# intellerce/controlanimate

Measured on AMD Instinct MI355X. Metric: frames_per_sec, higher is better.
Workload: dtype fp16

## Files before the change

controlanimate_amd/_capi.py:

```python
from __future__ import annotations

import ctypes as C
import os

_HERE = os.path.dirname(os.path.abspath(__file__))
LIB_PATH = os.environ.get("CA_HIP_LIB") or os.path.join(_HERE, "csrc", "libcontrolanimate_hip.so")

CA_BF16, CA_F16 = 0, 1
CA_F32 = 2
CA_ACT_NONE, CA_ACT_SILU = 0, 1
ABI_VERSION = 16


class CAHipUnavailable(RuntimeError):
    pass


class CAHipError(RuntimeError):
    pass


class GemmArgs(C.Structure):
    _fields_ = [
        ("a", C.c_void_p), ("a2", C.c_void_p), ("w", C.c_void_p), ("c", C.c_void_p),
# ... 162 lines not shown
                                         C.c_void_p, C.c_void_p, C.c_int32, C.c_int32, C.c_int32, C.c_int32,
                                         C.POINTER(C.c_float), C.c_float, C.c_void_p]),
    "ca_lincomb": (C.c_int, [C.c_void_p, C.POINTER(C.c_void_p), C.POINTER(C.c_float), C.c_int32, C.c_int64, C.c_void_p]),
    "ca_conv3x3_narrow": (C.c_int, [C.POINTER(ConvNarrowArgs), C.c_void_p]),
    "ca_conv3x3_narrow_plan_name": (C.c_int, [C.POINTER(ConvNarrowArgs), C.c_char_p, C.c_int32]),
    "ca_rgb8_to_nhwc": (C.c_int, [C.c_void_p, C.c_void_p, C.c_int32, C.c_int32, C.c_int32, C.c_int32, C.c_void_p]),
    "ca_resize_lanczos4_u8": (C.c_int, [C.c_void_p, C.c_void_p, C.c_int32, C.c_int32, C.c_int32, C.c_int32, C.c_int32,
                                         C.c_void_p, C.c_void_p, C.c_void_p, C.c_void_p, C.c_void_p]),
    "ca_color_match_workspace_bytes": (C.c_int64, [C.c_int32, C.c_int64]),
    "ca_hist_u8x3": (C.c_int, [C.c_void_p, C.c_void_p, C.c_int32, C.c_int64, C.c_void_p]),
    "ca_color_moments_f64": (C.c_int, [C.c_void_p, C.c_void_p, C.c_void_p, C.c_void_p, C.c_int32, C.c_int64, C.c_void_p, C.c_int64, C.c_void_p]),
    "ca_color_transform_f64": (C.c_int, [C.c_void_p, C.c_void_p, C.c_void_p, C.c_void_p, C.c_void_p, C.c_void_p, C.c_int32, C.c_int64, C.c_void_p]),
    "ca_sort_f64_segments": (C.c_int, [C.c_void_p, C.c_void_p, C.c_int32, C.c_int64, C.c_void_p, C.c_int64, C.c_void_p]),
    "ca_color_rank_map_f64": (C.c_int, [C.c_void_p, C.c_void_p, C.c_void_p, C.c_void_p, C.c_void_p, C.c_void_p, C.c_int32, C.c_int64,
                                         C.c_void_p, C.c_int64, C.c_void_p]),
    "ca_color_finish_u8": (C.c_int, [C.c_void_p, C.c_void_p, C.c_int32, C.c_int64, C.c_int32, C.c_void_p, C.c_int64, C.c_void_p]),
    "ca_canny_workspace_bytes": (C.c_int64, [C.c_int32, C.c_int32, C.c_int32]),
    "ca_canny_tile_w": (C.c_int32, []),
    "ca_canny_tile_h": (C.c_int32, []),
    "ca_canny_classify": (C.c_int, [C.c_void_p, C.c_int32, C.c_int32, C.c_int32, C.c_int32, C.c_int32, C.c_int32, C.c_void_p, C.c_int64, C.c_void_p]),
    "ca_canny_link": (C.c_int, [C.c_int32, C.c_int32, C.c_int32, C.c_void_p, C.c_int64, C.c_void_p]),
    "ca_canny_link_stage": (C.c_int, [C.c_int32, C.c_int32, C.c_int32, C.c_void_p, C.c_int64, C.c_int32, C.c_void_p]),
    "ca_canny_emit": (C.c_int, [C.c_int32, C.c_int32, C.c_int32, C.c_void_p, C.c_int64, C.c_void_p, C.c_void_p, C.c_int32, C.c_int32, C.c_void_p]),
}

_lib = None


def lib() -> C.CDLL:
    global _lib
    if _lib is not None:
        return _lib
    import torch
    if not os.path.exists(LIB_PATH):
        raise CAHipUnavailable(
            f"{LIB_PATH} is missing: the HIP extension is not built. Run "
            "`python -m controlanimate_amd._build` (needs hipcc); there is no CPU fallback.")
    try:
        handle = C.CDLL(LIB_PATH)
    except OSError as e:
        raise CAHipUnavailable(f"cannot load {LIB_PATH}: {e}") from e
    for name, (res, args) in SYMBOLS.items():
        fn = getattr(handle, name)
        fn.restype = res
        fn.argtypes = args
    if handle.ca_abi_version() != ABI_VERSION:
# ... 10 lines not shown
```

controlanimate_amd/context.py:

```python
from __future__ import annotations

from dataclasses import dataclass, field
from typing import Optional

import torch


@dataclass
class ExecCtx:
    b: int
    f: int
    dtype: torch.dtype
    temb: torch.Tensor
    emb_groups: int
    ehs: Optional[torch.Tensor] = None
    frames_per_kv: int = 1
    kv_mod: int = 0
    gn_frames_per_stat: int = 1
    cache: dict = field(default_factory=dict)

    @property
    def images(self) -> int:
        return self.b * self.f

    def rows_per_emb_group(self, h: int, w: int) -> int:
        return self.images // self.emb_groups * h * w


class Dispatch:
    gemm_ar = True
    ff_fused = True
    tattn_fused = True
    xattn_fused = True
    attn_out_fused = True
    xattn_ip_fused = True
    conv_winograd = True
    gn_winograd = True
    ln_row_sums = True
    repeat_kernel = True
    ln_fold = True
    cfg_shared = True
    cn_cfg_dedup = True
    controlnet_streams = 2


dispatch = Dispatch()
```

controlanimate_amd/csrc/ca_gemm.hip:

```cpp

#include "ca_gemm_core.h"

namespace {
using namespace ca_gemm_detail;
#include "ca_conv_wino.h"

template <int DT, int BM, int BN, int WAVES_M, int WAVES_N, int MODE>
__global__ __launch_bounds__(256) void k_gemm(GemmKParams p) {
  constexpr int TM = BM / WAVES_M / 16;
  constexpr int TN = BN / WAVES_N / 16;
  constexpr int AI = BM / 32;
  constexpr int BI = BN / 32;
  static_assert(2 * (BM + BN) * BK >= BM * (BN + 8), "epilogue staging must fit");
  __shared__ __attribute__((aligned(16))) u16 smem[2 * (BM + BN) * BK];

  const int tid = threadIdx.x;
  const int lane = tid & 63;
  const int wid = tid >> 6;
  const int wm = wid / WAVES_N, wn = wid % WAVES_N;
  const int g = lane >> 4, l15 = lane & 15;

  const int tiles_n = (p.n + BN - 1) / BN;
  const unsigned bid = xcd_remap(blockIdx.x, gridDim.x);
  int tile_m, tile_n;
// ... 875 lines not shown
  return CA_OK;
}

extern "C" int ca_conv3x3(const ca_conv_args* a, void* stream) {
  GemmKParams p{};
  int rc = conv_prepare(a, p);
  if (rc) return rc;
  hipStream_t st = (hipStream_t)stream;
  if (wino_taken(a)) {
    rc = launch_conv_wino(a, p, st);
    if (rc) return rc;
    CA_CHECK_LAUNCH("ca_conv3x3(winograd)");
    return CA_OK;
  }
  CA_REQUIRE(!a->x_is_wino_v, "ca_conv3x3: x_is_wino_v, but the Winograd route does not take these arguments (images=%d %dx%d cin=%d+%d cout=%d dtype=%d w_wino=%p "
             "workspace=%p of %lld bytes, needs %lld)", a->images, a->hin, a->win, a->cin1, a->cin2, a->cout, a->dtype, a->w_wino, a->workspace,
             (long long)a->workspace_bytes, (long long)wino_workspace_bytes(a));
  rc = a->dtype == CA_BF16 ? launch_gemm<CA_BF16, 1>(p, st) : launch_gemm<CA_F16, 1>(p, st);
  if (rc) return rc;
  CA_CHECK_LAUNCH("ca_conv3x3");
  return CA_OK;
}

extern "C" int ca_gemm_plan_name(const ca_gemm_args* a, char* buf, int32_t len) {
  CA_REQUIRE(buf && len > 0, "ca_gemm_plan_name: buffer");
  GemmKParams p{};
  int rc = gemm_prepare(a, p);
  if (rc) return rc;
  plan_label(plan_gemm(p, 0), buf, len);
  return CA_OK;
}

extern "C" int ca_conv3x3_plan_name(const ca_conv_args* a, char* buf, int32_t len) {
  CA_REQUIRE(buf && len > 0, "ca_conv3x3_plan_name: buffer");
  GemmKParams p{};
  int rc = conv_prepare(a, p);
  if (rc) return rc;
  if (wino_taken(a)) {
    snprintf(buf, (size_t)len, "wino_pq256x320");
    return CA_OK;
  }
  plan_label(plan_gemm(p, 1), buf, len);
  return CA_OK;
}
```

controlanimate_amd/csrc/ca_gemm_core.h:

```cpp
#pragma once
#include "ca_common.h"
#include <stdlib.h>

namespace ca_gemm_detail {


struct GemmKParams {
  const u16* a;
  const u16* a2;
  const u16* w;
  void* c;
  const float* bias;
  const float* rowbias;
  const float* ln_stats;
  const float* ln_colsum;
  const u16* res;
  int64_t lda, lda2, ldc, ld_res, ld_rowbias;
  unsigned a_bytes, a2_bytes, w_bytes;
  int m, n;
  int c1, c2;
  int taps;
  int kc_tiles;
  int hin, win, hout, wout, stride, ups, pad_lo;
  int rows_per_group;
  float alpha, post;
  int act, geglu, out_f32;
  int splits;
  float* partial;
  int dbg;
  int tap_inner;
  float* row_sums;
  int ln_parts;
  int ln_inline;
  float ln_eps;
  const u16* wf;
  int w_group_rows;
  unsigned w_group_stride;
};

constexpr int BK = 64;

constexpr int GROUP_M = 8;
__device__ __forceinline__ void tile_coords(unsigned bid, int tiles_m, int tiles_n, int& tile_m, int& tile_n) {
  const unsigned gsz = GROUP_M * tiles_n;
  const unsigned group = bid / gsz, in = bid - group * gsz;
  const int first_m = group * GROUP_M;
  const int gm = tiles_m - first_m < GROUP_M ? tiles_m - first_m : GROUP_M;
  tile_m = first_m + in % gm;
  tile_n = in / gm;
}

__device__ __forceinline__ void k_tile_split(const GemmKParams& p, int t, int kct, int& tap, int& cc) {
  if (p.taps == 1) {
    tap = 0;
    cc = t;
  } else if (p.tap_inner) {
    cc = t / p.taps;
    tap = t - cc * p.taps;
  } else {
    tap = t / kct;
// ... 281 lines not shown
        b += v.y;
      }
      *reinterpret_cast<float2*>(p.row_sums + ((int64_t)(m0 + tid) * (p.n / BN) + n0 / BN) * 2) = make_float2(a, b);
    }
  }
}


constexpr unsigned DMA_OOB = 0xFFFFFFF0u;

enum PlanKind {
  PK_WRES = 0,
  PK_PP2,
  PK_PP2_SPLITK,
  PK_DMA,
  PK_DMA_SPLITK,
  PK_REG,
  PK_PS,
  PK_PQ,
  PK_AR,
};

constexpr int64_t FIT31 = 0x7FFFFF00ll;
inline int64_t c_extent_bytes(const GemmKParams& p) { return (((int64_t)p.m - 1) * p.ldc + (p.geglu ? p.n / 2 : p.n)) * 2; }
inline int64_t res_extent_bytes(const GemmKParams& p) { return p.res ? (((int64_t)p.m - 1) * p.ld_res + p.n) * 2 : 0; }
inline bool act_out_fit31(const GemmKParams& p) {
  return c_extent_bytes(p) < FIT31 && res_extent_bytes(p) < FIT31 && p.a_bytes < FIT31 && (!p.c2 || p.a2_bytes < FIT31);
}

}

int ca_launch_gemm_pp(const ca_gemm_detail::GemmKParams& p, int dtype, int mode, ca_gemm_detail::PlanKind kind, unsigned tiles, hipStream_t st);
int ca_launch_gemm_ar(const ca_gemm_detail::GemmKParams& p, int dtype, hipStream_t st);
```

controlanimate_amd/csrc/ca_gemm_pp.hip:

```cpp
#include "ca_gemm_core.h"
#include <type_traits>

namespace {
using namespace ca_gemm_detail;
#include "ca_gemm_pp2.h"
#include "ca_gemm_wres.h"
#include "ca_gemm_ps.h"
#include "ca_gemm_pq.h"

int cu_count() {
  static int n = 0;
  if (!n) {
    int dev = 0;
    hipDeviceProp_t prop;
    if (hipGetDevice(&dev) == hipSuccess && hipGetDeviceProperties(&prop, dev) == hipSuccess) n = prop.multiProcessorCount;
    if (n <= 0) n = 256;
  }
  return n;
}

template <class Launch>
int launch_stamped(const GemmKParams& p, hipStream_t st, const char* label, unsigned sep, unsigned eol, Launch launch) {
  static unsigned long long* dbuf = nullptr;
  if (!dbuf && hipMalloc(&dbuf, 4096 * 8) != hipSuccess) return CA_ERR_LAUNCH;
// ... 43 lines not shown
#ifdef CA_STAMPS
      if (p.dbg == 9) return launch_stamped(p, st, "ps", 8, 10, launch);
#endif
      launch(p);
      return CA_OK;
    }
    case PK_WRES: {
      if (MODE != 0) return CA_ERR_LAUNCH;
      const int panels = p.n / 160;
      const int chunks = (p.m + 255) / 256;
      int per = (cu_count() / 8) / panels;
      if (per * 8 > chunks) per = chunks / 8;
      if (per < 1) per = 1;
      const unsigned rb_bytes = p.rowbias ? (unsigned)(((int64_t)((p.m - 1) / p.rows_per_group) * p.ld_rowbias + p.n) * 4) : 16u;
      hipLaunchKernelGGL((k_gemm_wres<DT>), dim3(8 * per * panels), dim3(512), 0, st, p, panels, 8 * per, chunks, rb_bytes, c_bytes, res_bytes);
      return CA_OK;
    }
    case PK_PP2:
      hipLaunchKernelGGL((k_gemm_pp2<DT, MODE>), dim3(tiles), dim3(512), 0, st, p);
      return CA_OK;
    default: return CA_ERR_LAUNCH;
  }
}
}

int ca_launch_gemm_pp(const ca_gemm_detail::GemmKParams& p0, int dtype, int mode, ca_gemm_detail::PlanKind kind, unsigned tiles, hipStream_t st) {
  static const int dbg = CA_KNOB("CA_PP_DBG", 0);
  ca_gemm_detail::GemmKParams p = p0;
  p.dbg = dbg;
  if (dtype == CA_BF16) return mode ? launch_pp<CA_BF16, 1>(p, kind, tiles, st) : launch_pp<CA_BF16, 0>(p, kind, tiles, st);
  return mode ? launch_pp<CA_F16, 1>(p, kind, tiles, st) : launch_pp<CA_F16, 0>(p, kind, tiles, st);
}
```

controlanimate_amd/csrc/ca_gemm_pq.h:

```cpp

#ifdef CA_PQ_ABLATE
#define CA_PQ_ABL(bit) (((CA_PQ_ABLATE) & (bit)) != 0)
#else
#define CA_PQ_ABL(bit) false
#endif

template <int DT, int MODE, int EPI = 0>
__global__ __launch_bounds__(512, 2) void k_gemm_pq(GemmKParams p, int tiles_total, unsigned c_bytes, unsigned res_bytes) {
  constexpr int BM = 256, BN = 320, KT = 64;
  constexpr int TM = 8, TN = 5;
  constexpr int A_ROWS = 256, B0_ROWS = 128, B1_ROWS = 192;
  constexpr int OFF_A = 0, OFF_B0 = A_ROWS * KT, OFF_B1 = (A_ROWS + B0_ROWS) * KT;
  constexpr int BUF = (A_ROWS + B0_ROWS + B1_ROWS) * KT;
  constexpr int PAR_BASE = 2 * BUF * 2;
  constexpr int P_BI = 0, P_RB0 = 1280, P_RB1 = 2560, P_CS = 3840, PSET = EPI == 1 ? 5120 : 4096;
  constexpr int FLAG_BASE = PAR_BASE + 2 * PSET;
  constexpr int SMEM_BYTES = FLAG_BASE + 8 * 2 * 256;
  static_assert(SMEM_BYTES <= 160 * 1024, "LDS");
  __shared__ __attribute__((aligned(16))) unsigned char smem_b[SMEM_BYTES];
  u16* const smem = reinterpret_cast<u16*>(smem_b);

  const int tid = threadIdx.x;
  const int lane = tid & 63;
  const int wid = __builtin_amdgcn_readfirstlane(tid >> 6);
  const int wr = wid >> 2, wc = wid & 3;
  const int g = lane >> 4, l15 = lane & 15;

  const int tiles_n = p.n / BN;
  const int tiles_m = (p.m + BM - 1) / BM;
  const int G = gridDim.x;
  const int bslot = (G % 8 == 0) ? (int)(blockIdx.x % 8) * (G / 8) + (int)(blockIdx.x / 8) : (int)blockIdx.x;
  const int my_tiles = bslot < tiles_total ? (tiles_total - bslot + G - 1) / G : 0;
  if (my_tiles == 0) return;

  for (int i = tid; i < 8 * 2 * 64; i += 512) reinterpret_cast<unsigned*>(smem_b + FLAG_BASE)[i] = 0xFFFFFFFFu;
  __syncthreads();

  const __amdgpu_buffer_rsrc_t rs_a = __builtin_amdgcn_make_buffer_rsrc((void*)p.a, 0, p.a_bytes, 0x00020000);
  const __amdgpu_buffer_rsrc_t rs_a2 = __builtin_amdgcn_make_buffer_rsrc((void*)(p.a2 ? p.a2 : p.a), 0, p.a2 ? p.a2_bytes : p.a_bytes, 0x00020000);
  const __amdgpu_buffer_rsrc_t rs_w = __builtin_amdgcn_make_buffer_rsrc((void*)p.w, 0, p.w_bytes, 0x00020000);
  const __amdgpu_buffer_rsrc_t rs_c = __builtin_amdgcn_make_buffer_rsrc(p.c, 0, c_bytes, 0x00020000);
  const __amdgpu_buffer_rsrc_t rs_bi = __builtin_amdgcn_make_buffer_rsrc((void*)(p.bias ? (const void*)p.bias : (const void*)p.w), 0, p.bias ? (unsigned)p.n * 4u : 0u, 0x00020000);
  const bool geglu = EPI == 1 && p.geglu != 0;
  const unsigned long long res_addr = (unsigned long long)(p.res ? (const void*)p.res : (const void*)p.c);
  const u32x4 rs_res = {(unsigned)__builtin_amdgcn_readfirstlane((int)(unsigned)res_addr), (unsigned)__builtin_amdgcn_readfirstlane((int)(unsigned)((res_addr >> 32) & 0xffffu)),
                        (unsigned)__builtin_amdgcn_readfirstlane((int)(p.res ? res_bytes : 0u)), 0x00020000u};
  const unsigned rb_groups = p.rowbias ? (unsigned)((p.m + p.rows_per_group - 1) / p.rows_per_group) : 0u;
  const __amdgpu_buffer_rsrc_t rs_rb = __builtin_amdgcn_make_buffer_rsrc((void*)(p.rowbias ? (const void*)p.rowbias : (const void*)p.w), 0,
                                                                         p.rowbias ? (unsigned)(((int64_t)(rb_groups - 1) * p.ld_rowbias + p.n) * 4) : 0u, 0x00020000);
  const __amdgpu_buffer_rsrc_t rs_seq = __builtin_amdgcn_make_buffer_rsrc((void*)ca_seq_table.v, 0, 4096u, 0x00020000);

#ifdef CA_STAMPS
// ... 20 lines not shown
  unsigned b0_v[2] = {0, 0}, b1_v[3] = {0, 0, 0};
  unsigned a_v[4] = {0, 0, 0, 0};
  int d_seq = 0, d_t = 0, d_tap = 0, d_c0 = 0, d_n = 0;
  bool d_live = true;
  unsigned char* const my_flags = smem_b + FLAG_BASE + wid * 2 * 256;

  auto tile_of = [&](int seq, int& tm, int& tn) __attribute__((always_inline)) -> bool {
    const int id = seq * G + bslot;
    if (id >= tiles_total) return false;
    tile_coords((unsigned)id, tiles_m, tiles_n, tm, tn);
    return true;
  };

  auto dma_set_tile = [&](int seq, int m0, int n0) __attribute__((always_inline)) {
    if (CA_PQ_ABL(16)) m0 = 0, n0 = 0;
    int lane_o = lane;
    asm volatile("" : "+v"(lane_o));
    const int r8 = lane_o >> 3, cp = lane_o & 7;
    const int a_chunk0 = cp ^ swz(r8), b1_chunk0 = cp ^ swz(wid * 24 + r8);
#pragma unroll
    for (int i = 0; i < 4; ++i) {
      const int m = m0 + wid * 32 + i * 8 + r8;
      const bool ok = m < p.m;
      if (MODE == 1) {
        const int mm = ok ? m : p.m - 1;
        const int hw = p.hout * p.wout;
        const int img = mm / hw;
        const int rem = mm - img * hw;
        const int ho = rem / p.wout, wo = rem - ho * p.wout;
        const int hi0 = ho * p.stride - p.pad_lo, wi0 = wo * p.stride - p.pad_lo;
        const int p0 = (img * p.hin + hi0) * p.win + wi0;
        a_v[i] = ((unsigned)p0 & 0xFFFFFFu) | (hi0 >= 0 ? 1u << 24 : 0u) | (hi0 + 2 < p.hin ? 1u << 25 : 0u) | (wi0 >= 0 ? 1u << 26 : 0u) | (wi0 + 2 < p.win ? 1u << 27 : 0u) |
                 (ok ? 1u << 28 : 0u);
      } else {
        a_v[i] = ok ? (unsigned)m * (unsigned)p.lda * 2u + (unsigned)((a_chunk0 ^ (4 * (i & 1))) * 16) : OOB_V;
      }
    }
    unsigned wgrp = 0u;
    if (MODE == 0 && EPI == 0 && p.w_group_rows > 0) wgrp = (unsigned)(m0 / p.w_group_rows) * p.w_group_stride;
#pragma unroll
    for (int i = 0; i < 2; ++i) {
      const int r = wid * 16 + i * 8 + r8;
      b0_v[i] = wgrp + (unsigned)(n0 + (r >> 5) * 80 + ca_ps_col((r >> 4) & 1, r & 15, geglu)) * wld * 2u + (unsigned)((a_chunk0 ^ (4 * i)) * 16);
    }
#pragma unroll
    for (int i = 0; i < 3; ++i) {
      const int r1 = wid * 24 + i * 8 + r8;
      b1_v[i] = wgrp + (unsigned)(n0 + (r1 / 48) * 80 + ca_ps_col(2 + (r1 % 48) / 16, r1 & 15, geglu)) * wld * 2u + (unsigned)((b1_chunk0 ^ (4 * (i & 1))) * 16);
    }
    d_tap = 0;
    d_c0 = 0;
    unsigned char* pset = smem_b + PAR_BASE + (seq & 1) * PSET;
    if (EPI == 1 && wid == 4) {
      const __amdgpu_buffer_rsrc_t rs_cs = __builtin_amdgcn_make_buffer_rsrc((void*)(p.ln_colsum ? (const void*)p.ln_colsum : (const void*)p.w), 0, p.ln_colsum ? (unsigned)p.n * 4u : 0u, 0x00020000);
      __builtin_amdgcn_raw_ptr_buffer_load_lds(rs_cs, (__attribute__((address_space(3))) void*)(pset + P_CS), 16, (unsigned)n0 * 4u + lane_o * 16u, 0, 0, 0);
      __builtin_amdgcn_raw_ptr_buffer_load_lds(rs_cs, (__attribute__((address_space(3))) void*)(pset + P_CS + 1024), 4, (unsigned)n0 * 4u + 1024u + lane_o * 4u, 0, 0, 0);
    }
    if (wid >= 1 && wid <= 3) {
      const bool has1 = p.rowbias && m0 / p.rows_per_group + 1 < (int)rb_groups;
      const unsigned base = wid == 1 ? (unsigned)n0 * 4u
                                     : wid == 2 ? (unsigned)n0 * 4u + (unsigned)(p.rowbias ? m0 / p.rows_per_group : 0) * (unsigned)p.ld_rowbias * 4u
                                                : (has1 ? (unsigned)n0 * 4u + (unsigned)(m0 / p.rows_per_group + 1) * (unsigned)p.ld_rowbias * 4u : OOB_V);
// ... 1 lines not shown
      if (wid == 1) {
        __builtin_amdgcn_raw_ptr_buffer_load_lds(rs_bi, (__attribute__((address_space(3))) void*)dst, 16, base + lane_o * 16u, 0, 0, 0);
        __builtin_amdgcn_raw_ptr_buffer_load_lds(rs_bi, (__attribute__((address_space(3))) void*)(dst + 1024), 4, base + 1024u + lane_o * 4u, 0, 0, 0);
      } else {
        __builtin_amdgcn_raw_ptr_buffer_load_lds(rs_rb, (__attribute__((address_space(3))) void*)dst, 16, base + lane_o * 16u, 0, 0, 0);
        __builtin_amdgcn_raw_ptr_buffer_load_lds(rs_rb, (__attribute__((address_space(3))) void*)(dst + 1024), 4, base + 1024u + lane_o * 4u, 0, 0, 0);
      }
    }
  };

  auto issue_tile = [&]() __attribute__((always_inline)) {
    if (!d_live) return;
    if (CA_PQ_ABL(1) && d_n >= 2) {
      ++d_n;
      ++d_t;
      return;
    }
    const int par = d_n & 1;
    u16* buf = smem + par * BUF;
    const unsigned wk = (unsigned)(d_tap * kc + d_c0) * 2u;
    const bool src2 = d_c0 >= p.c1;
    __builtin_amdgcn_raw_ptr_buffer_load_lds(rs_w, (__attribute__((address_space(3))) void*)(buf + OFF_B0 + (wid * 2 + 0) * 8 * KT), 16, b0_v[0], wk, 0, 0);
    __builtin_amdgcn_raw_ptr_buffer_load_lds(rs_w, (__attribute__((address_space(3))) void*)(buf + OFF_B0 + (wid * 2 + 1) * 8 * KT), 16, b0_v[1], wk, 0, 0);
    if (MODE == 1) {
      int lane_o = lane;
      asm volatile("" : "+v"(lane_o));
      const unsigned cs2 = (unsigned)(src2 ? p.c2 : p.c1) * 2u;
      const int kh = d_tap >= 6 ? 2 : (d_tap >= 3 ? 1 : 0), kw = d_tap - kh * 3;
      const unsigned need = (1u << 28) | (kh == 0 ? 1u << 24 : kh == 2 ? 1u << 25 : 0u) | (kw == 0 ? 1u << 26 : kw == 2 ? 1u << 27 : 0u);
      const int delta = kh * p.win + kw;
      const unsigned cadd = (unsigned)(src2 ? d_c0 - p.c1 : d_c0) * 2u + (unsigned)(((lane_o & 7) ^ swz(lane_o >> 3)) * 16);
#pragma unroll
      for (int i = 0; i < 4; ++i) {
        const unsigned av = a_v[i];
        const int pix = (((int)(av << 8)) >> 8) + delta;
        const unsigned off = __umul24((unsigned)pix, cs2) + (cadd ^ ((i & 1) ? 64u : 0u));
        const unsigned voff = (av & need) == need ? off : OOB_V;
        void* d = buf + OFF_A + (wid * 4 + i) * 8 * KT;
        if (src2) __builtin_amdgcn_raw_ptr_buffer_load_lds(rs_a2, (__attribute__((address_space(3))) void*)d, 16, voff, 0, 0, 0);
        else __builtin_amdgcn_raw_ptr_buffer_load_lds(rs_a, (__attribute__((address_space(3))) void*)d, 16, voff, 0, 0, 0);
      }
    } else {
#pragma unroll
      for (int i = 0; i < 4; ++i)
        __builtin_amdgcn_raw_ptr_buffer_load_lds(rs_a, (__attribute__((address_space(3))) void*)(buf + OFF_A + (wid * 4 + i) * 8 * KT), 16, a_v[i], (unsigned)d_c0 * 2u, 0, 0);
    }
#pragma unroll
    for (int i = 0; i < 3; ++i)
      __builtin_amdgcn_raw_ptr_buffer_load_lds(rs_w, (__attribute__((address_space(3))) void*)(buf + OFF_B1 + (wid * 3 + i) * 8 * KT), 16, b1_v[i], wk, 0, 0);
    __builtin_amdgcn_raw_ptr_buffer_load_lds(rs_seq, (__attribute__((address_space(3))) void*)(my_flags + par * 256), 4, 0u, (unsigned)(d_n & 1023) * 4u, 0, 0);
    ++d_n;
    ++d_t;
// ... 83 lines not shown
#pragma unroll
    for (int i = 0; i < TM; ++i)
#pragma unroll
      for (int j = 0; j < TN; ++j) acc[i][j] = Elem<DT>::mfma(fb[j], fa[i], acc[i][j]);
    __builtin_amdgcn_s_setprio(0);
    __builtin_amdgcn_sched_barrier(0);
  };

  auto epilogue = [&](int seq, int m0, int n0) __attribute__((always_inline)) {
    const unsigned char* pset = smem_b + PAR_BASE + (seq & 1) * PSET;
    int lane_o = lane;
    asm volatile("" : "+v"(lane_o));
    const int l15 = lane_o & 15, g = lane_o >> 4;
    int rb_sel = 0;
    if (p.rowbias) rb_sel = (m0 + wr * 128) / p.rows_per_group - m0 / p.rows_per_group;
    const unsigned char* rbp = pset + (rb_sel ? P_RB1 : P_RB0);
    f32x4 bi[TN], rb[TN];
#pragma unroll
    for (int j = 0; j < TN; ++j) {
      const int c0 = wc * 80 + (j < 4 ? 32 * (j >> 1) + 8 * g + 4 * (j & 1) : 64 + 4 * g);
      bi[j] = *reinterpret_cast<const f32x4*>(pset + P_BI + c0 * 4);
      rb[j] = *reinterpret_cast<const f32x4*>(rbp + c0 * 4);
    }
    auto rowoff_of = [&](int i, int64_t ld) __attribute__((always_inline)) -> unsigned {
      const int m = m0 + wr * 128 + i * 16 + l15;
      return m < p.m ? (unsigned)m * (unsigned)ld * 2u + (unsigned)(n0 + wc * 80) * 2u : OOB_V;
    };
    u32x4 r16[2][2];
    u32x2 r8[2];
    r16[0][0] = r16[0][1] = r16[1][0] = r16[1][1] = (u32x4){0u, 0u, 0u, 0u};
    r8[0] = r8[1] = (u32x2){0u, 0u};
    auto res_load = [&](int i, int slot) __attribute__((always_inline)) {
      const unsigned ro = rowoff_of(i, p.ld_res);
      const unsigned o0 = ro + (unsigned)(8 * g) * 2u, o1 = ro + (unsigned)(32 + 8 * g) * 2u, o2 = ro + (unsigned)(64 + 4 * g) * 2u;
      asm volatile("s_nop 4\n\tbuffer_load_dwordx4 %0, %3, %6, 0 offen\n\tbuffer_load_dwordx4 %1, %4, %6, 0 offen\n\tbuffer_load_dwordx2 %2, %5, %6, 0 offen"
                   : "=&v"(r16[slot][0]), "=&v"(r16[slot][1]), "=&v"(r8[slot])
                   : "v"(o0), "v"(o1), "v"(o2), "s"(rs_res)
                   : "memory");
    };
    float rsum[TM], rsq[TM];
#pragma unroll
    for (int i = 0; i < TM; ++i) rsum[i] = rsq[i] = 0.f;
    if (p.res) res_load(0, 0);
#pragma unroll
    for (int i = 0; i < TM; ++i) {
      const int slot = i & 1;
      if (p.res) {
        if (i + 1 < TM) res_load(i + 1, slot ^ 1);
        if (i == 0 || i + 1 == TM) asm volatile("s_waitcnt vmcnt(3)" ::: "memory");
// ... 106 lines not shown
          const unsigned lo = pack2<DT>(v[0], v[1]), hi = pack2<DT>(v[2], v[3]);
          if ((j & 1) == 0) {
            w[0] = lo;
            w[1] = hi;
          } else {
            __builtin_amdgcn_raw_buffer_store_b128((u32x4){w[0], w[1], lo, hi}, rs_c, ro + (unsigned)(32 * (j >> 1) + 8 * g) * 2u, 0, 0);
          }
        } else {
          __builtin_amdgcn_raw_buffer_store_b64((u32x2){pack2<DT>(v[0], v[1]), pack2<DT>(v[2], v[3])}, rs_c, ro + (unsigned)(64 + 4 * g) * 2u, 0, 0);
        }
      }
      if (geglu) {
        __builtin_amdgcn_raw_buffer_store_b128((u32x4){w[0], w[1], w[2], w[3]}, rs_c, ro + (unsigned)(8 * g) * 2u, 0, 0);
        __builtin_amdgcn_raw_buffer_store_b32(w[4], rs_c, ro + (unsigned)(32 + 2 * g) * 2u, 0, 0);
      }
    }
#pragma unroll
    for (int i = 0; i < TM; ++i)
#pragma unroll
      for (int j = 0; j < TN; ++j) acc[i][j] = (f32x4){0.f, 0.f, 0.f, 0.f};
    asm volatile("s_waitcnt lgkmcnt(0)" ::: "memory");
  };

  const bool g1_late = MODE == 1 && wr == 1;
  CA_PQ_SET_TILE(0)
  issue_tile();
  if (g1_late) advance_and_issue();
  {
    const unsigned f0 = flag_begin(0);
    flag_finish(0, 0, f0);
  }
  __builtin_amdgcn_s_barrier();
  if (wr == 1) __builtin_amdgcn_s_barrier();

  int cv = 0;
  for (int seq = 0; seq < my_tiles; ++seq) {
    int tm, tn;
    tile_of(seq, tm, tn);
    const int m0 = tm * BM, n0 = tn * BN;
    for (int t = 0; t < (p.dbg == 2 ? 0 : nt); ++t) {
      const int par = cv & 1;
      const u16* buf = smem + par * BUF;
      stamp(1);
      __builtin_amdgcn_sched_barrier(0);
      read_frags(buf, 0);
      if (!g1_late) advance_and_issue();
      asm volatile("s_waitcnt lgkmcnt(0)" ::: "memory");
// ... 35 lines not shown
```

controlanimate_amd/kernels.py:

```python
from __future__ import annotations

import ctypes as C
from typing import Optional

import torch

from . import _capi
from .context import dispatch
from ._capi import (AttnArgs, ConvArgs, ConvNarrowArgs, FfArgs, TattnArgs, XattnArgs, GemmArgs, GroupNormArgs, LayerNormArgs, CA_ACT_NONE,
                    CA_ACT_SILU, CA_BF16, CA_F16, check, lib)

ACT_NONE, ACT_SILU = CA_ACT_NONE, CA_ACT_SILU
ACT_QUICK_GELU, ACT_GELU = 2, 3


def dt_code(dtype: torch.dtype) -> int:
    if dtype == torch.bfloat16:
        return CA_BF16
    if dtype == torch.float16:
        return CA_F16
    raise TypeError(f"activations must be bf16 or fp16, got {dtype}")


def _stream() -> int:
# ... 251 lines not shown
        ld_res = cout
    if rowbias is not None:
        assert rowbias.dtype == torch.float32 and rowbias.dim() == 2 and rowbias.shape[1] == cout and rows_per_group > 0
    if bias is not None:
        assert bias.dtype == torch.float32 and bias.numel() == cout
    args = ConvArgs(x=_p(x), x2=_p(x2), w=_p(w), y=_p(y), bias=_p(bias), rowbias=_p(rowbias),
                    residual=_p(residual), ld_res=ld_res,
                    ld_rowbias=rowbias.stride(0) if rowbias is not None else 0, images=images, hin=hin,
                    win=win, cin1=cin1, cin2=cin2, cout=cout, stride=stride, upsample=int(upsample),
                    rows_per_group=rows_per_group, alpha=alpha, post_scale=post_scale, act=act,
                    out_f32=int(out_f32), dtype=dt_code(x.dtype), pad_asym=int(pad_asym))
    if w_wino is not None and dispatch.conv_winograd:
        assert w_wino.dtype == x.dtype and w_wino.is_contiguous() and tuple(w_wino.shape) == (16, cout, cin1 + cin2)
        args.w_wino = _p(w_wino)
    wbytes = int(lib().ca_conv3x3_workspace_bytes(C.byref(args)))
    if wbytes > 0:
        ws = torch.empty((wbytes,), device=x.device, dtype=torch.uint8)
        args.workspace, args.workspace_bytes = _p(ws), wbytes
    _record_plan(lib().ca_conv3x3_plan_name, args)
    check(lib().ca_conv3x3(C.byref(args), _stream()), "ca_conv3x3")
    return y


_gn_wino_declined: dict = {}


def group_norm_conv3x3_wino(x: torch.Tensor, gamma: torch.Tensor, beta: torch.Tensor, w: torch.Tensor, w_wino: torch.Tensor, *,
                            x2: Optional[torch.Tensor] = None, groups: int = 32, eps: float = 1e-5, act: int = ACT_NONE,
                            bias: Optional[torch.Tensor] = None, rowbias: Optional[torch.Tensor] = None, rows_per_group: int = 0,
                            residual: Optional[torch.Tensor] = None, post_scale: float = 1.0) -> Optional[torch.Tensor]:
    if not (dispatch.conv_winograd and dispatch.gn_winograd):
        return None
    _req_cuda(x, gamma, beta, w, w_wino, x2, bias, rowbias, residual)
    if x.dim() != 4 or not x.is_contiguous() or x.dtype != torch.float16 or (x2 is not None and (not x2.is_contiguous() or x2.shape[:3] != x.shape[:3])):
        return None
    images, h, w_, c1 = x.shape
    c2 = 0 if x2 is None else x2.shape[3]
    c, cout = c1 + c2, w.shape[0]
    tiles = images * (h // 2) * (w_ // 2)
    key = (images, h, w_, c1, c2, cout, groups, act, rowbias is not None, residual is not None, rows_per_group)
    if _gn_wino_declined.get(key):
        return None
    cargs = ConvArgs(x=_p(x), x2=None, w=_p(w), y=_p(x), bias=_p(bias), rowbias=_p(rowbias), residual=_p(residual),
                     ld_res=cout if residual is not None else 0, ld_rowbias=rowbias.stride(0) if rowbias is not None else 0, images=images, hin=h,
                     win=w_, cin1=c, cin2=0, cout=cout, stride=1, upsample=0, rows_per_group=rows_per_group, alpha=1.0, post_scale=post_scale,
                     act=ACT_NONE, out_f32=0, dtype=dt_code(x.dtype), pad_asym=0, w_wino=_p(w_wino), x_is_wino_v=1)
# ... 438 lines not shown
```

controlanimate_amd/layers.py:

```python
from __future__ import annotations

from typing import Callable, List, Optional, Sequence, Tuple

import torch
from torch import nn

from . import kernels as K
from .context import dispatch

ALIGN = 256


class Packed:

    __slots__ = ("shape", "dtype", "fill", "offset", "t", "frag")

    def __init__(self, shape, dtype, fill):
        self.shape = tuple(int(s) for s in shape)
        self.dtype = dtype
        self.fill = fill
        self.offset = -1
        self.t: Optional[torch.Tensor] = None
        self.frag = None

# ... 112 lines not shown

    def run(self, a: torch.Tensor, **kw) -> torch.Tensor:
        return K.gemm(a, self.w.t, bias=None if self.b is None else self.b.t, **kw)


class HipConv1x1(nn.Module):

    def __init__(self, in_channels: int, out_channels: int):
        super().__init__()
        self.in_channels, self.out_channels = in_channels, out_channels
        self.weight = nn.Parameter(torch.empty(out_channels, in_channels, 1, 1))
        self.bias = nn.Parameter(torch.zeros(out_channels))
        nn.init.normal_(self.weight, std=in_channels ** -0.5)
        self.w = self.b = None

    def pack(self, arena: WeightArena, dtype):
        self.w = arena.add((self.out_channels, self.in_channels), dtype, lambda: _f32(self.weight).reshape(self.out_channels, self.in_channels))
        self.b = arena.add((self.out_channels,), torch.float32, lambda: _f32(self.bias))

    def run(self, a: torch.Tensor, **kw) -> torch.Tensor:
        return K.gemm(a, self.w.t, bias=self.b.t, **kw)


class HipConv3x3(nn.Module):

    def __init__(self, in_channels: int, out_channels: int, stride: int = 1):
        super().__init__()
        self.in_channels, self.out_channels, self.stride = in_channels, out_channels, stride
        self.cin_pad = (in_channels + 7) // 8 * 8
        self.weight = nn.Parameter(torch.empty(out_channels, in_channels, 3, 3))
        self.bias = nn.Parameter(torch.zeros(out_channels))
        nn.init.normal_(self.weight, std=(9 * in_channels) ** -0.5)
        self.w = self.b = None
        self.winograd = True

    def _packed_weight(self) -> torch.Tensor:
        w = _f32(self.weight).permute(0, 2, 3, 1)
        if self.cin_pad != self.in_channels:
            w = torch.nn.functional.pad(w, (0, self.cin_pad - self.in_channels))
        return w.contiguous()

    def _winograd_weight(self) -> torch.Tensor:
        g = torch.tensor([[1.0, 0.0, 0.0], [0.5, 0.5, 0.5], [0.5, -0.5, 0.5], [0.0, 0.0, 1.0]], dtype=torch.float32, device=self.weight.device)
        u = torch.einsum("xk,oikl,yl->xyoi", g, _f32(self.weight), g)
        return u.reshape(16, self.out_channels, self.in_channels).contiguous()

    def pack(self, arena: WeightArena, dtype):
        self.w = arena.add((self.out_channels, 3, 3, self.cin_pad), dtype, self._packed_weight)
        self.b = arena.add((self.out_channels,), torch.float32, lambda: _f32(self.bias))
        self.u = None
        if (dispatch.conv_winograd and self.stride == 1 and self.winograd and self.in_channels >= 640 and self.in_channels % 64 == 0
                and self.out_channels % 320 == 0):
            self.u = arena.add((16, self.out_channels, self.in_channels), dtype, self._winograd_weight)

    def run(self, x: torch.Tensor, **kw) -> torch.Tensor:
        u = getattr(self, "u", None)
        return K.conv3x3(x, self.w.t, bias=self.b.t, stride=self.stride, w_wino=None if u is None else u.t, **kw)


class HipGroupNorm(nn.Module):
    def __init__(self, num_groups: int, num_channels: int, eps: float = 1e-5):
        super().__init__()
        self.num_groups, self.num_channels, self.eps = num_groups, num_channels, eps
        self.weight = nn.Parameter(torch.ones(num_channels))
        self.bias = nn.Parameter(torch.zeros(num_channels))
        self.g = self.b = None

    def pack(self, arena: WeightArena, dtype):
        self.g = arena.add((self.num_channels,), torch.float32, lambda: _f32(self.weight))
        self.b = arena.add((self.num_channels,), torch.float32, lambda: _f32(self.bias))

    def run(self, x: torch.Tensor, *, x2: Optional[torch.Tensor] = None, frames_per_stat: int = 1, act: int = K.ACT_NONE):
        return K.group_norm(x, self.g.t, self.b.t, x2=x2, groups=self.num_groups, frames_per_stat=frames_per_stat,
                            eps=self.eps, act=act)


class HipLayerNorm(nn.Module):
    def __init__(self, dim: int, eps: float = 1e-5):
# ... 74 lines not shown
```

controlanimate_amd/resnet.py:

```python
from __future__ import annotations

from typing import Optional

import torch
from torch import nn

from . import kernels as K
from .context import ExecCtx
from .layers import HipConv1x1, HipConv3x3, HipGroupNorm, HipLinear, WeightArena


class InflatedConv3d(HipConv3x3):
    """3x3 (stride 1/2) per-frame convolution; parameters as nn.Conv2d."""


class InflatedGroupNorm(HipGroupNorm):
    """GroupNorm with per-frame statistics (v2) -- or cross-frame when the model says so (v1)."""


class Upsample3D(nn.Module):
    def __init__(self, channels, use_conv=True, out_channels=None, name="conv"):
        super().__init__()
        self.channels, self.out_channels = channels, out_channels or channels
        self.conv = InflatedConv3d(channels, self.out_channels)

    def pack(self, arena, dtype):
        self.conv.pack(arena, dtype)

    def forward(self, x: torch.Tensor) -> torch.Tensor:
        return self.conv.run(x, upsample=True)


class Downsample3D(nn.Module):
    def __init__(self, channels, use_conv=True, out_channels=None, padding=1, name="conv"):
        super().__init__()
        self.channels, self.out_channels = channels, out_channels or channels
        self.conv = InflatedConv3d(channels, self.out_channels, stride=2)

    def pack(self, arena, dtype):
        self.conv.pack(arena, dtype)

    def forward(self, x: torch.Tensor) -> torch.Tensor:
        return self.conv.run(x)


class ResnetBlock3D(nn.Module):
    def __init__(self, *, in_channels, out_channels=None, temb_channels=512, groups=32, eps=1e-6,
# ... 45 lines not shown
```

include/controlanimate_hip.h:

```cpp
#ifndef CONTROLANIMATE_HIP_H
#define CONTROLANIMATE_HIP_H

#include <stdint.h>

#ifdef __cplusplus
extern "C" {
#endif

#define CA_ABI_VERSION 16

#define CA_BF16 0
#define CA_F16 1
#define CA_F32 2

#define CA_OK 0
#define CA_ERR_INVALID_ARG (-1)
#define CA_ERR_UNSUPPORTED (-2)
#define CA_ERR_LAUNCH (-3)

#define CA_ACT_NONE 0
#define CA_ACT_SILU 1
#define CA_ACT_QUICK_GELU 2
#define CA_ACT_GELU 3

// ... 109 lines not shown
  void* y;
  const float* bias;
  const float* rowbias;
  const void* residual;
  int64_t ld_res, ld_rowbias;
  int32_t images, hin, win, cin1, cin2, cout;
  int32_t stride;
  int32_t upsample;
  int32_t rows_per_group;
  float alpha, post_scale;
  int32_t act;
  int32_t out_f32;
  int32_t dtype;
  void* workspace;
  int64_t workspace_bytes;
  int32_t pad_asym;
  const void* w_wino;
  int32_t x_is_wino_v;
} ca_conv_args;
int ca_pack_w_wino(const void* w, int32_t cout, int32_t cin, int32_t dtype, void* dst, void* stream);
int64_t ca_conv3x3_workspace_bytes(const ca_conv_args* args);
int ca_conv3x3(const ca_conv_args* args, void* stream);
int ca_conv3x3_plan_name(const ca_conv_args* args, char* buf, int32_t len);

typedef struct ca_groupnorm_args {
  const void* x;
  const void* x2;
  void* y;
  const float* gamma;
  const float* beta;
  float* partials;
  int32_t images, hw, c1, c2;
  int32_t groups;
  int32_t frames_per_stat;
  float eps;
  int32_t act;
  int32_t dtype;
  void* wino_v;
  int32_t wino_h, wino_w;
} ca_groupnorm_args;
int ca_groupnorm_wino_supported(const ca_groupnorm_args* args);
int64_t ca_groupnorm_partials_floats(int32_t images, int32_t hw, int32_t frames_per_stat, int32_t groups);
int ca_groupnorm_stats(const ca_groupnorm_args* args, void* stream);
int ca_groupnorm_apply(const ca_groupnorm_args* args, void* stream);
int ca_groupnorm(const ca_groupnorm_args* args, void* stream);

// ... 132 lines not shown
```

Baseline: 16.22.

## Fold nearest-2x upsample into conv as four 2x2 phase convolutions

Adds a sub-pixel phase path for the upsampler's 3x3 conv. Because nearest 2x upsampling followed by a 3x3 conv is equivalent to four 2x2 convolutions on the low-resolution input (one per output phase), weights are precombined into four 2x2 kernels and the persistent PQ GEMM gets a MODE 2 that gathers low-res source pixels and scatters results to interleaved output positions. This cuts the conv's multiply-adds from 9 taps to 4 taps per output pixel and avoids reading upsampled input, at the cost of an extra packed weight tensor and extra index arithmetic per row.

```diff
diff --git a/controlanimate_amd/_capi.py b/controlanimate_amd/_capi.py
--- a/controlanimate_amd/_capi.py
+++ b/controlanimate_amd/_capi.py
@@ -208,6 +208,9 @@
     "ca_canny_link": (C.c_int, [C.c_int32, C.c_int32, C.c_int32, C.c_void_p, C.c_int64, C.c_void_p]),
     "ca_canny_link_stage": (C.c_int, [C.c_int32, C.c_int32, C.c_int32, C.c_void_p, C.c_int64, C.c_int32, C.c_void_p]),
     "ca_canny_emit": (C.c_int, [C.c_int32, C.c_int32, C.c_int32, C.c_void_p, C.c_int64, C.c_void_p, C.c_void_p, C.c_int32, C.c_int32, C.c_void_p]),
+    "ca_conv_up2_phase_supported": (C.c_int, [C.POINTER(ConvArgs)]),
+    "ca_conv_up2_phase": (C.c_int, [C.POINTER(ConvArgs), C.c_void_p]),
+    "ca_conv_up2_phase_plan_name": (C.c_int, [C.POINTER(ConvArgs), C.c_char_p, C.c_int32]),
 }
 
 _lib = None
diff --git a/controlanimate_amd/context.py b/controlanimate_amd/context.py
--- a/controlanimate_amd/context.py
+++ b/controlanimate_amd/context.py
@@ -36,6 +36,7 @@
     xattn_ip_fused = True
     conv_winograd = True
     gn_winograd = True
+    conv_up2_phase = True
     ln_row_sums = True
     repeat_kernel = True
     ln_fold = True
diff --git a/controlanimate_amd/csrc/ca_gemm.hip b/controlanimate_amd/csrc/ca_gemm.hip
--- a/controlanimate_amd/csrc/ca_gemm.hip
+++ b/controlanimate_amd/csrc/ca_gemm.hip
@@ -921,6 +921,72 @@
   return CA_OK;
 }
 
+static bool up2_capable(const ca_conv_args* a, GemmKParams& p) {
+  if (!a || !a->x || !a->w || !a->y || a->x2 || a->cin2 != 0 || a->images <= 0 || a->hin <= 0 || a->win <= 0) return false;
+  if (a->upsample != 1 || a->stride != 1 || a->pad_asym || a->out_f32 || a->x_is_wino_v || a->rowbias) return false;
+  if ((a->dtype != CA_F16 && a->dtype != CA_BF16) || a->act != CA_ACT_NONE || a->post_scale != 1.f) return false;
+  if (a->cin1 <= 0 || a->cin1 % BK != 0 || a->cout <= 0 || a->cout % 320 != 0) return false;
+  if ((((uintptr_t)a->x | (uintptr_t)a->w | (uintptr_t)a->y | (uintptr_t)a->residual) & 15) != 0) return false;
+  if (a->residual && (a->ld_res < a->cout || a->ld_res % 8 != 0)) return false;
+  const int64_t rows = (int64_t)a->images * a->hin * a->win;
+  if (rows + a->win + 2 >= (1 << 23)) return false;
+  p = GemmKParams{};
+  p.a = (const u16*)a->x;
+  p.w = (const u16*)a->w;
+  p.c = a->y;
+  p.bias = a->bias;
+  p.res = (const u16*)a->residual;
+  p.ldc = a->cout;
+  p.ld_res = a->ld_res;
+  p.a_bytes = desc_bytes(rows * a->cin1);
+  p.w_bytes = desc_bytes((int64_t)4 * a->cout * 4 * a->cin1);
+  p.n = a->cout;
+  p.c1 = a->cin1;
+  p.taps = 4;
+  p.tap_inner = 1;
+  p.kc_tiles = a->cin1 / BK;
+  p.hin = a->hin, p.win = a->win, p.hout = 2 * a->hin, p.wout = 2 * a->win;
+  p.stride = 1, p.ups = 1, p.pad_lo = 1;
+  p.rows_per_group = 1;
+  p.alpha = a->alpha, p.post = 1.f;
+  p.splits = 1;
+  p.up2_rows = (int)rows;
+  p.up2_tiles = ceil_div_i((int)rows, 256);
+  p.m = 4 * p.up2_tiles * 256;
+  p.up2_mag_w = a->win == 1 ? 0xFFFFFFFFu : (unsigned)((1ull << 32) / (unsigned)a->win);
+  p.up2_mag_h = a->hin == 1 ? 0xFFFFFFFFu : (unsigned)((1ull << 32) / (unsigned)a->hin);
+  p.w_group_stride = (unsigned)((int64_t)a->cout * 4 * a->cin1 * 2);
+  return p.a_bytes && p.w_bytes && act_out_fit31(p) && p.w_bytes < FIT31;
+}
+inline unsigned up2_tiles_total(const GemmKParams& p) { return (unsigned)(4 * p.up2_tiles * (p.n / 320)); }
+inline bool up2_pays(const GemmKParams& p) {
+  const unsigned tiles = up2_tiles_total(p);
+  return tiles >= 256 && (tiles % 256 == 0 || tiles >= 1024);
+}
+
+extern "C" int ca_conv_up2_phase_supported(const ca_conv_args* a) {
+  GemmKParams p{};
+  return up2_capable(a, p) && up2_pays(p) ? 1 : 0;
+}
+
+extern "C" int ca_conv_up2_phase(const ca_conv_args* a, void* stream) {
+  GemmKParams p{};
+  CA_REQUIRE(up2_capable(a, p), "ca_conv_up2_phase: arguments the phase form does not take (one fp16 / bf16 source with cin %% 64 == 0, cout %% 320 == 0, upsample = 1, "
+             "stride 1, symmetric padding, no row bias / activation / post scale / fp32 output, 16-byte aligned operands, < 2^23 source pixels)");
+  int rc = ca_launch_gemm_pp(p, a->dtype, 2, PK_PQ, up2_tiles_total(p), (hipStream_t)stream);
+  if (rc) return rc;
+  CA_CHECK_LAUNCH("ca_conv_up2_phase");
+  return CA_OK;
+}
+
+extern "C" int ca_conv_up2_phase_plan_name(const ca_conv_args* a, char* buf, int32_t len) {
+  CA_REQUIRE(buf && len > 0, "ca_conv_up2_phase_plan_name: buffer");
+  GemmKParams p{};
+  CA_REQUIRE(up2_capable(a, p), "ca_conv_up2_phase_plan_name: arguments the phase form does not take");
+  snprintf(buf, (size_t)len, "up2_pq256x320");
+  return CA_OK;
+}
+
 extern "C" int ca_gemm_plan_name(const ca_gemm_args* a, char* buf, int32_t len) {
   CA_REQUIRE(buf && len > 0, "ca_gemm_plan_name: buffer");
   GemmKParams p{};
diff --git a/controlanimate_amd/csrc/ca_gemm_core.h b/controlanimate_amd/csrc/ca_gemm_core.h
--- a/controlanimate_amd/csrc/ca_gemm_core.h
+++ b/controlanimate_amd/csrc/ca_gemm_core.h
@@ -36,6 +36,8 @@
   const u16* wf;
   int w_group_rows;
   unsigned w_group_stride;
+  int up2_rows, up2_tiles;
+  unsigned up2_mag_w, up2_mag_h;
 };
 
 constexpr int BK = 64;
@@ -363,8 +365,9 @@
 };
 
 constexpr int64_t FIT31 = 0x7FFFFF00ll;
-inline int64_t c_extent_bytes(const GemmKParams& p) { return (((int64_t)p.m - 1) * p.ldc + (p.geglu ? p.n / 2 : p.n)) * 2; }
-inline int64_t res_extent_bytes(const GemmKParams& p) { return p.res ? (((int64_t)p.m - 1) * p.ld_res + p.n) * 2 : 0; }
+inline int64_t out_rows(const GemmKParams& p) { return p.up2_rows ? 4 * (int64_t)p.up2_rows : (int64_t)p.m; }
+inline int64_t c_extent_bytes(const GemmKParams& p) { return ((out_rows(p) - 1) * p.ldc + (p.geglu ? p.n / 2 : p.n)) * 2; }
+inline int64_t res_extent_bytes(const GemmKParams& p) { return p.res ? ((out_rows(p) - 1) * p.ld_res + p.n) * 2 : 0; }
 inline bool act_out_fit31(const GemmKParams& p) {
   return c_extent_bytes(p) < FIT31 && res_extent_bytes(p) < FIT31 && p.a_bytes < FIT31 && (!p.c2 || p.a2_bytes < FIT31);
 }
diff --git a/controlanimate_amd/csrc/ca_gemm_pp.hip b/controlanimate_amd/csrc/ca_gemm_pp.hip
--- a/controlanimate_amd/csrc/ca_gemm_pp.hip
+++ b/controlanimate_amd/csrc/ca_gemm_pp.hip
@@ -89,12 +89,21 @@
     default: return CA_ERR_LAUNCH;
   }
 }
+
+template <int DT>
+int launch_up2(const GemmKParams& p, PlanKind kind, unsigned tiles, hipStream_t st) {
+  if (kind != PK_PQ) return CA_ERR_LAUNCH;
+  const unsigned grid = tiles < (unsigned)cu_count() ? tiles : (unsigned)cu_count();
+  hipLaunchKernelGGL((k_gemm_pq<DT, 2>), dim3(grid), dim3(512), 0, st, p, (int)tiles, (unsigned)c_extent_bytes(p), (unsigned)res_extent_bytes(p));
+  return CA_OK;
+}
 }
 
 int ca_launch_gemm_pp(const ca_gemm_detail::GemmKParams& p0, int dtype, int mode, ca_gemm_detail::PlanKind kind, unsigned tiles, hipStream_t st) {
   static const int dbg = CA_KNOB("CA_PP_DBG", 0);
   ca_gemm_detail::GemmKParams p = p0;
   p.dbg = dbg;
+  if (mode == 2) return dtype == CA_BF16 ? launch_up2<CA_BF16>(p, kind, tiles, st) : launch_up2<CA_F16>(p, kind, tiles, st);
   if (dtype == CA_BF16) return mode ? launch_pp<CA_BF16, 1>(p, kind, tiles, st) : launch_pp<CA_BF16, 0>(p, kind, tiles, st);
   return mode ? launch_pp<CA_F16, 1>(p, kind, tiles, st) : launch_pp<CA_F16, 0>(p, kind, tiles, st);
 }
diff --git a/controlanimate_amd/csrc/ca_gemm_pq.h b/controlanimate_amd/csrc/ca_gemm_pq.h
--- a/controlanimate_amd/csrc/ca_gemm_pq.h
+++ b/controlanimate_amd/csrc/ca_gemm_pq.h
@@ -4,6 +4,11 @@
 #else
 #define CA_PQ_ABL(bit) false
 #endif
+
+__device__ __forceinline__ unsigned pq_udiv(unsigned r, unsigned d, unsigned mag) {
+  const unsigned q = __umulhi(r, mag);
+  return r - q * d >= d ? q + 1 : q;
+}
 
 template <int DT, int MODE, int EPI = 0>
 __global__ __launch_bounds__(512, 2) void k_gemm_pq(GemmKParams p, int tiles_total, unsigned c_bytes, unsigned res_bytes) {
@@ -27,7 +32,7 @@
   const int g = lane >> 4, l15 = lane & 15;
 
   const int tiles_n = p.n / BN;
-  const int tiles_m = (p.m + BM - 1) / BM;
+  const int tiles_m = MODE == 2 ? 4 * p.up2_tiles : (p.m + BM - 1) / BM;
   const int G = gridDim.x;
   const int bslot = (G % 8 == 0) ? (int)(blockIdx.x % 8) * (G / 8) + (int)(blockIdx.x / 8) : (int)blockIdx.x;
   const int my_tiles = bslot < tiles_total ? (tiles_total - bslot + G - 1) / G : 0;
@@ -94,7 +99,20 @@
     for (int i = 0; i < 4; ++i) {
       const int m = m0 + wid * 32 + i * 8 + r8;
       const bool ok = m < p.m;
-      if (MODE == 1) {
+      if (MODE == 2) {
+        const int ph = m0 / (p.up2_tiles * BM);
+        const int py = ph >> 1, px = ph & 1;
+        const int r = m - ph * (p.up2_tiles * BM);
+        const bool okr = r < p.up2_rows;
+        const int rr = okr ? r : p.up2_rows - 1;
+        const unsigned q = pq_udiv((unsigned)rr, (unsigned)p.win, p.up2_mag_w);
+        const int xs = rr - (int)q * p.win;
+        const int ys = (int)q - (int)pq_udiv(q, (unsigned)p.hin, p.up2_mag_h) * p.hin;
+        const int hi0 = ys + py - 1, wi0 = xs + px - 1;
+        const int p0 = rr + (py - 1) * p.win + (px - 1);
+        a_v[i] = ((unsigned)p0 & 0xFFFFFFu) | (hi0 >= 0 ? 1u << 24 : 0u) | (hi0 + 1 < p.hin ? 1u << 25 : 0u) | (wi0 >= 0 ? 1u << 26 : 0u) | (wi0 + 1 < p.win ? 1u << 27 : 0u) |
+                 (okr ? 1u << 28 : 0u);
+      } else if (MODE == 1) {
         const int mm = ok ? m : p.m - 1;
         const int hw = p.hout * p.wout;
         const int img = mm / hw;
@@ -110,6 +128,7 @@
     }
     unsigned wgrp = 0u;
     if (MODE == 0 && EPI == 0 && p.w_group_rows > 0) wgrp = (unsigned)(m0 / p.w_group_rows) * p.w_group_stride;
+    if (MODE == 2) wgrp = (unsigned)(m0 / (p.up2_tiles * BM)) * p.w_group_stride;
 #pragma unroll
     for (int i = 0; i < 2; ++i) {
       const int r = wid * 16 + i * 8 + r8;
@@ -157,12 +176,13 @@
     const bool src2 = d_c0 >= p.c1;
     __builtin_amdgcn_raw_ptr_buffer_load_lds(rs_w, (__attribute__((address_space(3))) void*)(buf + OFF_B0 + (wid * 2 + 0) * 8 * KT), 16, b0_v[0], wk, 0, 0);
     __builtin_amdgcn_raw_ptr_buffer_load_lds(rs_w, (__attribute__((address_space(3))) void*)(buf + OFF_B0 + (wid * 2 + 1) * 8 * KT), 16, b0_v[1], wk, 0, 0);
-    if (MODE == 1) {
+    if (MODE != 0) {
       int lane_o = lane;
       asm volatile("" : "+v"(lane_o));
       const unsigned cs2 = (unsigned)(src2 ? p.c2 : p.c1) * 2u;
-      const int kh = d_tap >= 6 ? 2 : (d_tap >= 3 ? 1 : 0), kw = d_tap - kh * 3;
-      const unsigned need = (1u << 28) | (kh == 0 ? 1u << 24 : kh == 2 ? 1u << 25 : 0u) | (kw == 0 ? 1u << 26 : kw == 2 ? 1u << 27 : 0u);
+      const int kh = MODE == 2 ? d_tap >> 1 : (d_tap >= 6 ? 2 : (d_tap >= 3 ? 1 : 0)), kw = MODE == 2 ? d_tap & 1 : d_tap - kh * 3;
+      const unsigned need = MODE == 2 ? (1u << 28) | (kh == 0 ? 1u << 24 : 1u << 25) | (kw == 0 ? 1u << 26 : 1u << 27)
+                                      : (1u << 28) | (kh == 0 ? 1u << 24 : kh == 2 ? 1u << 25 : 0u) | (kw == 0 ? 1u << 26 : kw == 2 ? 1u << 27 : 0u);
       const int delta = kh * p.win + kw;
       const unsigned cadd = (unsigned)(src2 ? d_c0 - p.c1 : d_c0) * 2u + (unsigned)(((lane_o & 7) ^ swz(lane_o >> 3)) * 16);
 #pragma unroll
@@ -292,9 +312,15 @@
       bi[j] = *reinterpret_cast<const f32x4*>(pset + P_BI + c0 * 4);
       rb[j] = *reinterpret_cast<const f32x4*>(rbp + c0 * 4);
     }
+    const int up_ph = MODE == 2 ? m0 / (p.up2_tiles * BM) : 0;
     auto rowoff_of = [&](int i, int64_t ld) __attribute__((always_inline)) -> unsigned {
-      const int m = m0 + wr * 128 + i * 16 + l15;
-      return m < p.m ? (unsigned)m * (unsigned)ld * 2u + (unsigned)(n0 + wc * 80) * 2u : OOB_V;
+      int m = m0 + wr * 128 + i * 16 + l15;
+      if (MODE == 2) {
+        const int r = m - up_ph * (p.up2_tiles * BM);
+        const int xs = r - (int)pq_udiv((unsigned)r, (unsigned)p.win, p.up2_mag_w) * p.win;
+        m = r < p.up2_rows ? 4 * r - 2 * xs + (up_ph >> 1) * 2 * p.win + (up_ph & 1) : 0x7FFFFFFF;
+      }
+      return m < (MODE == 2 ? 4 * p.up2_rows : p.m) ? (unsigned)m * (unsigned)ld * 2u + (unsigned)(n0 + wc * 80) * 2u : OOB_V;
     };
     u32x4 r16[2][2];
     u32x2 r8[2];
@@ -447,7 +473,7 @@
     asm volatile("s_waitcnt lgkmcnt(0)" ::: "memory");
   };
 
-  const bool g1_late = MODE == 1 && wr == 1;
+  const bool g1_late = MODE != 0 && wr == 1;
   CA_PQ_SET_TILE(0)
   issue_tile();
   if (g1_late) advance_and_issue();
diff --git a/controlanimate_amd/kernels.py b/controlanimate_amd/kernels.py
--- a/controlanimate_amd/kernels.py
+++ b/controlanimate_amd/kernels.py
@@ -297,6 +297,39 @@
     return y
 
 
+def _up2_args(x, w_phase, bias, residual, alpha, y=None) -> ConvArgs:
+    images, hin, win, cin = x.shape
+    cout = w_phase.shape[1]
+    return ConvArgs(x=_p(x), w=_p(w_phase), y=_p(y) if y is not None else _p(x), bias=_p(bias), residual=_p(residual),
+                    ld_res=cout if residual is not None else 0, images=images, hin=hin, win=win, cin1=cin, cin2=0, cout=cout, stride=1,
+                    upsample=1, rows_per_group=0, alpha=alpha, post_scale=1.0, act=ACT_NONE, out_f32=0, dtype=dt_code(x.dtype), pad_asym=0)
+
+
+def conv_up2_phase_supported(x: torch.Tensor, w_phase: torch.Tensor, *, bias: Optional[torch.Tensor] = None,
+                             residual: Optional[torch.Tensor] = None, alpha: float = 1.0) -> bool:
+    if x.dim() != 4 or w_phase.dim() != 5 or not x.is_contiguous() or x.dtype not in (torch.float16, torch.bfloat16):
+        return False
+    return bool(lib().ca_conv_up2_phase_supported(C.byref(_up2_args(x, w_phase, bias, residual, alpha))))
+
+
+def conv_up2_phase(x: torch.Tensor, w_phase: torch.Tensor, *, bias: Optional[torch.Tensor] = None,
+                   residual: Optional[torch.Tensor] = None, alpha: float = 1.0) -> torch.Tensor:
+    _req_cuda(x, w_phase, bias, residual)
+    assert x.dim() == 4 and x.is_contiguous() and w_phase.dim() == 5 and w_phase.is_contiguous() and w_phase.dtype == x.dtype
+    images, hin, win, cin = x.shape
+    cout = w_phase.shape[1]
+    assert tuple(w_phase.shape) == (4, cout, 2, 2, cin)
+    y = torch.empty((images, 2 * hin, 2 * win, cout), device=x.device, dtype=x.dtype)
+    if residual is not None:
+        assert residual.dtype == x.dtype and residual.is_contiguous() and residual.numel() == y.numel()
+    if bias is not None:
+        assert bias.dtype == torch.float32 and bias.numel() == cout
+    args = _up2_args(x, w_phase, bias, residual, alpha, y)
+    _record_plan(lib().ca_conv_up2_phase_plan_name, args)
+    check(lib().ca_conv_up2_phase(C.byref(args), _stream()), "ca_conv_up2_phase")
+    return y
+
+
 _gn_wino_declined: dict = {}
 
 
diff --git a/controlanimate_amd/layers.py b/controlanimate_amd/layers.py
--- a/controlanimate_amd/layers.py
+++ b/controlanimate_amd/layers.py
@@ -158,6 +158,12 @@
         return K.gemm(a, self.w.t, bias=self.b.t, **kw)
 
 
+def phase_weights(w: torch.Tensor) -> torch.Tensor:
+    sel = torch.tensor([[[1.0, 0.0, 0.0], [0.0, 1.0, 1.0]], [[1.0, 1.0, 0.0], [0.0, 0.0, 1.0]]], dtype=w.dtype, device=w.device)
+    wp = torch.einsum("ydk,xel,oikl->yxodei", sel, sel, w)
+    return wp.reshape(4, w.shape[0], 2, 2, w.shape[1]).contiguous()
+
+
 class HipConv3x3(nn.Module):
 
     def __init__(self, in_channels: int, out_channels: int, stride: int = 1):
@@ -169,6 +175,7 @@
         nn.init.normal_(self.weight, std=(9 * in_channels) ** -0.5)
         self.w = self.b = None
         self.winograd = True
+        self.up2_phase = False
 
     def _packed_weight(self) -> torch.Tensor:
         w = _f32(self.weight).permute(0, 2, 3, 1)
@@ -188,8 +195,16 @@
         if (dispatch.conv_winograd and self.stride == 1 and self.winograd and self.in_channels >= 640 and self.in_channels % 64 == 0
                 and self.out_channels % 320 == 0):
             self.u = arena.add((16, self.out_channels, self.in_channels), dtype, self._winograd_weight)
+        self.wp = None
+        if dispatch.conv_up2_phase and self.up2_phase and self.stride == 1 and self.in_channels % 64 == 0 and self.out_channels % 320 == 0:
+            self.wp = arena.add((4, self.out_channels, 2, 2, self.in_channels), dtype, lambda: phase_weights(_f32(self.weight)))
 
     def run(self, x: torch.Tensor, **kw) -> torch.Tensor:
+        wp = getattr(self, "wp", None)
+        if wp is not None and dispatch.conv_up2_phase and kw.get("upsample") and set(kw) <= {"upsample", "residual", "alpha"}:
+            ph = {k: v for k, v in kw.items() if k != "upsample"}
+            if K.conv_up2_phase_supported(x, wp.t, bias=self.b.t, **ph):
+                return K.conv_up2_phase(x, wp.t, bias=self.b.t, **ph)
         u = getattr(self, "u", None)
         return K.conv3x3(x, self.w.t, bias=self.b.t, stride=self.stride, w_wino=None if u is None else u.t, **kw)
 
diff --git a/controlanimate_amd/resnet.py b/controlanimate_amd/resnet.py
--- a/controlanimate_amd/resnet.py
+++ b/controlanimate_amd/resnet.py
@@ -23,6 +23,7 @@
         super().__init__()
         self.channels, self.out_channels = channels, out_channels or channels
         self.conv = InflatedConv3d(channels, self.out_channels)
+        self.conv.up2_phase = True
 
     def pack(self, arena, dtype):
         self.conv.pack(arena, dtype)
diff --git a/include/controlanimate_hip.h b/include/controlanimate_hip.h
--- a/include/controlanimate_hip.h
+++ b/include/controlanimate_hip.h
@@ -155,6 +155,9 @@
 int64_t ca_conv3x3_workspace_bytes(const ca_conv_args* args);
 int ca_conv3x3(const ca_conv_args* args, void* stream);
 int ca_conv3x3_plan_name(const ca_conv_args* args, char* buf, int32_t len);
+int ca_conv_up2_phase_supported(const ca_conv_args* args);
+int ca_conv_up2_phase(const ca_conv_args* args, void* stream);
+int ca_conv_up2_phase_plan_name(const ca_conv_args* args, char* buf, int32_t len);
 
 typedef struct ca_groupnorm_args {
   const void* x;
```

Result: faster. 16.43, median of 6 (+1.3%).
